# yinan-codes/Rossby-wave-ray-tracing

Measured on AMD Instinct MI355X. Metric: ray-steps/sec (whole node), 10^6 rays RKF45; max |Δpos| vs CPU ref, higher is better.
Workload: dtype f64

## Files before the change

include/rwrt.h:

```cpp
#ifndef RWRT_H
#define RWRT_H

#include <stdint.h>

#ifdef __cplusplus
extern "C" {
#endif

#define RWRT_ABI_VERSION 5
#define RWRT_NFIELD_REF 18
#define RWRT_NFIELD_PACK 12
#define RWRT_NVAR 5
#define RWRT_NMERC 12
#define RWRT_NOUT 8
#define RWRT_NSTATE 12

typedef enum {
  RWRT_OK = 0,
  RWRT_ERR_ARG = 1,
  RWRT_ERR_HIP = 2,
  RWRT_SOLVER_FAILED = 3
} rwrt_status;

typedef struct {
// ... 8 lines not shown
  double atol;
  double min_step;
  double cut_off;
  int32_t nt;
  int32_t reserved;
  double tstep;
} rwrt_params;

typedef struct {
  const void* d_levels;
  int32_t nlev;
  int32_t fp32;
  double t0;
  double dt;
} rwrt_background;
const char* rwrt_version(void);

typedef struct rwrt_ctx rwrt_ctx;
rwrt_status rwrt_ctx_create(int32_t device, rwrt_ctx** out);
rwrt_status rwrt_ctx_destroy(rwrt_ctx* ctx);
rwrt_status rwrt_ctx_set_latency_density(rwrt_ctx* ctx, int32_t rays_per_wave);
rwrt_status rwrt_ctx_set_tv_lanes(rwrt_ctx* ctx, int32_t lanes);
rwrt_status rwrt_ctx_set_handoff(rwrt_ctx* ctx, int32_t max_rays);
rwrt_status rwrt_ctx_set_trace(rwrt_ctx* ctx, int64_t* d_trace, int64_t capacity);
const char* rwrt_last_error(void);

rwrt_status rwrt_pack_fields(const rwrt_grid* g, const double* d_fields,
                             double* d_packed, void* stream);

rwrt_status rwrt_mercator_point(const rwrt_grid* g, const double* d_packed,
                                int64_t n, const double* d_lon,
                                const double* d_lat, double* d_out,
                                void* stream);

rwrt_status rwrt_rhs(const rwrt_grid* g, const double* d_packed, int64_t n,
                     const double* d_y, double* d_dydt, void* stream);

rwrt_status rwrt_dp54_attempt(const rwrt_grid* g, const double* d_packed,
                              int64_t n, const double* d_y, const double* d_f,
                              const double* d_h, double rtol, double atol,
                              double* d_K, double* d_ynew, double* d_err,
                              void* stream);

rwrt_status rwrt_ray_initial(const rwrt_grid* g, const double* d_packed,
                             int64_t nsource, const double* d_src_lon,
                             const double* d_src_lat, const double* d_src_cos,
// ... 246 lines not shown
```

rossby-wave-ray-tracing_amd/_hip.py:

```python
import ctypes
import os

import torch

_HERE = os.path.dirname(os.path.abspath(__file__))
LIB_PATH = os.environ.get("RWRT_LIB", os.path.join(_HERE, "librwrt.so"))

NFIELD_REF, NFIELD_PACK, NVAR, NMERC, NOUT, NSTATE = 18, 12, 5, 12, 8, 12
ABI_SYMBOLS = ("rwrt_version", "rwrt_last_error", "rwrt_ctx_create", "rwrt_ctx_destroy",
               "rwrt_ctx_set_latency_density", "rwrt_ctx_set_tv_lanes", "rwrt_ctx_set_handoff",
               "rwrt_ctx_set_trace",
               "rwrt_pack_fields",
               "rwrt_mercator_point", "rwrt_rhs", "rwrt_dp54_attempt",
               "rwrt_ray_initial", "rwrt_rk45_init", "rwrt_rk45_run", "rwrt_rk45_run_tails",
               "rwrt_expand_tails", "rwrt_row_slots", "rwrt_rk45_run_slots", "rwrt_expand_slots",
               "rwrt_launch_plan_bytes", "rwrt_launch_plan",
               "rwrt_rk4_run", "rwrt_ray_density", "rwrt_ray_summary", "rwrt_ray_arrival", "rwrt_ray_flux",
               "rwrt_ray_track", "rwrt_ray_cross",
               "rwrt_wn_map", "rwrt_wn_fill",
               "rwrt_sh_filter",
               "rwrt_bs_ready", "rwrt_bs_diag", "rwrt_rk45_init_tv", "rwrt_rk45_run_tv", "rwrt_rk45_run_tv_tails",
               "rwrt_rk45_run_tv_slots", "rwrt_rhs_tv",
               "rwrt_rk45_init_stack", "rwrt_rk45_run_stack",
               "rwrt_kat_rk45", "rwrt_selftest_math", "rwrt_host_fill_rows")

RWRT_OK, RWRT_ERR_ARG, RWRT_ERR_HIP, RWRT_SOLVER_FAILED = 0, 1, 2, 3
PLAN_SINCE, PLAN_TOTAL = 0, 1


class RwrtError(RuntimeError):
    pass


class SolverFailed(RwrtError):
# ... 129 lines not shown
        "rwrt_ray_track": [T, _I64, _I32, _I32, _P, _P, _P, _P, _P, _I64, _P, _P, _P, _P, _P, _P, _P],
        "rwrt_ray_cross": [X, _I64, _I32, _I32, _P, _P, _P, _P, _P, _I64, _P, _P, _P, _P, _P, _P, _P, _P, _P],
        "rwrt_ray_summary": [_I64, _I32, _I32, _P, _P, _P, _P, _P, _I64, R, _P, _P, _P],
        "rwrt_wn_map": [G, _P, _I32, _I64, _I32, _P, _P, _P, _I32, _P, _P, _P, _P, _P, _P, _P],
        "rwrt_wn_fill": [_I32, _I32, _I32, _I32, _P, _P, _P],
        "rwrt_sh_filter": [_I32, _I32, _I32, _I32, _P, _P, _P, _P, _P, _P, _P, _P],
        "rwrt_bs_ready": [_I32, _I32, _P, _P, _P, _D, _D, _P, _P, _I32, _P],
        "rwrt_bs_diag": [_I32, _I32, _I32, _P, _P, _P, _D, _D, ctypes.c_uint32, _P, _P, _I32, _P],
        "rwrt_rk45_init_tv": [G, B, _I64, _P, Pr, _P, _P, _P, _P, _P, _P],
        "rwrt_rk45_run_tv": [_P, G, B, _I64, Pr, _P, _I32, _I32, _P, _I64, _P, _P, _P, _P, _P, _P],
        "rwrt_rk45_run_tv_tails": [_P, G, B, _I64, Pr, _P, _I32, _I32, _P, _I64, _P, _P, _P, _P, _P, _P, _P,
                                   _P],
        "rwrt_rk45_run_tv_slots": [_P, G, B, _I64, Pr, _P, _I32, _I32, _P, _I64, _P, _P, _P, _P, _P, _P, _P,
                                   _P, _P],
        "rwrt_rk45_init_stack": [G, ctypes.POINTER(Stack), _I64, _P, Pr, _P, _P, _P, _P, _P, _P],
        "rwrt_rk45_run_stack": [_P, G, ctypes.POINTER(Stack), _I64, Pr, _P, _I32, _I32, _P, _P, _P, _P, _P, _P, _P,
                                _P, _P, _P],
        "rwrt_ctx_create": [_I32, ctypes.POINTER(_P)],
        "rwrt_ctx_destroy": [_P],
        "rwrt_ctx_set_latency_density": [_P, _I32],
        "rwrt_ctx_set_tv_lanes": [_P, _I32],
        "rwrt_ctx_set_handoff": [_P, _I32],
        "rwrt_ctx_set_trace": [_P, _P, _I64],
        "rwrt_rhs_tv": [G, B, _I64, _P, _P, _P, _P],
        "rwrt_kat_rk45": [_I32, _I64, _P, _I32, _P, _D, _D, _D, _P, _P],
        "rwrt_selftest_math": [_I32, _I64, _P, _P, _P, _P],
        "rwrt_host_fill_rows": [_P, _I64, _I64, _I64, _P, _P, _I64, _I64, _P],
    }
    for name, args in sig.items():
        fn = getattr(lib, name, None)
        if fn is None:
            continue
        fn.argtypes = args
        fn.restype = ctypes.c_int
    _lib = lib
    return lib


def version():
    return load().rwrt_version().decode()


def check(status):
    if status != RWRT_OK:
        msg = load().rwrt_last_error().decode()
        raise RwrtError(f"rwrt status {status}: {msg}")
# ... 29 lines not shown
        idx = self.device.index if self.device.index is not None else torch.cuda.current_device()
        h = _P()
        check(load().rwrt_ctx_create(int(idx), ctypes.byref(h)))
        self._h = h

    @property
    def handle(self):
        return self._h

    def set_latency_density(self, rays_per_wave):
        if getattr(self, "_qpw", 16) != int(rays_per_wave):
            check(load().rwrt_ctx_set_latency_density(self._h, int(rays_per_wave)))
            self._qpw = int(rays_per_wave)

    def set_tv_lanes(self, lanes):
        if getattr(self, "_tvl", 64) != int(lanes):
            check(load().rwrt_ctx_set_tv_lanes(self._h, int(lanes)))
            self._tvl = int(lanes)

    def set_handoff(self, max_rays):
        if getattr(self, "_hof", 16) != int(max_rays):
            check(load().rwrt_ctx_set_handoff(self._h, int(max_rays)))
            self._hof = int(max_rays)

    def set_trace(self, trace=None):
        if trace is None:
            check(load().rwrt_ctx_set_trace(self._h, None, 0))
        else:
            check(load().rwrt_ctx_set_trace(self._h, ctypes.c_void_p(trace.data_ptr()), int(trace.shape[0])))
        self._trace = trace

    _plan_scratch = None
    _plan_rays = 0

    def launch_plan(self, nray, total, state, count, prev_work, work, order, row_slot, nslot):
        lib = load()
        if self._plan_scratch is None or self._plan_rays < nray:
            need = _I64()
            check(lib.rwrt_launch_plan_bytes(int(nray), ctypes.byref(need)))
            self._plan_scratch = torch.empty(need.value, dtype=torch.uint8, device=self.device)
            self._plan_rays = int(nray)
        n_live = _I64()
        i64 = torch.int64
        check(lib.rwrt_launch_plan(int(nray), PLAN_TOTAL if total else PLAN_SINCE, dptr(state), dptr(count, i64),
                                   dptr(prev_work, i64), dptr(work, i64), dptr(order, i64),
                                   dptr(row_slot, torch.int32), dptr(nslot, i64), ctypes.byref(n_live),
# ... 14 lines not shown
```

rossby-wave-ray-tracing_amd/csrc/rwrt.hip:

```cpp

#include <hip/hip_runtime.h>

#include <cmath>
#include <cstdint>
#include <cstdlib>
#include <cstdio>
#include <cstring>
#include <mutex>
#include <string>
#include <type_traits>

#include "rwrt.h"
#include "nproots.h"

#ifdef RWRT_ANALYZE_HOT
__device__ __forceinline__ bool rwrt_rare_sink(bool c) {
  asm volatile("; rare %0" ::"s"(__builtin_amdgcn_ballot_w64(c)));
  return false;
}
#define RARE(c) rwrt_rare_sink(c)
#else
#define RARE(c) (c)
#endif
#ifdef RWRT_ANALYZE_MARK
#define MARK(name) do { __builtin_amdgcn_sched_barrier(0); asm volatile("; @MARK " name); __builtin_amdgcn_sched_barrier(0); } while (0)
#else
#define MARK(name)
#endif

#include "ray_point.h"
#include "stack_image.h"

namespace rwrt {

constexpr double kREarth = 6.3712e6;
constexpr double kOmega = 7.2921e-5;

__device__ __forceinline__ double div_rearth(double x) { return x / kREarth; }

#ifndef RWRT_ROW_NT
#define RWRT_ROW_NT 0
#endif
typedef double v2f64 __attribute__((ext_vector_type(2)));
template <bool NT>
__device__ __forceinline__ void store_row16(double2* o, double2 v) {
  if (NT) {
    v2f64 w;
    w.x = v.x;
    w.y = v.y;
    __builtin_nontemporal_store(w, reinterpret_cast<v2f64*>(o));
  } else {
    *o = v;
  }
// ... 2091 lines not shown
  int32_t handoff = 16;
};

template <class BG>
__device__ __forceinline__ double* row_block(const RunArgs<BG>& a, int64_t ray) {
  const int64_t slot = a.row_slot ? (int64_t)a.row_slot[ray] : ray;
  return slot < 0 ? nullptr : a.out + (size_t)slot * (size_t)(a.it_end - a.it_begin) * RWRT_NOUT;
}


__device__ __forceinline__ void store_tail(double* tail_row, int64_t ray, double2 r0, double2 r1, double2 r2,
                                           double2 r3) {
  double2* o = reinterpret_cast<double2*>(tail_row + (size_t)ray * RWRT_NOUT);
  o[0] = r0;
  o[1] = r1;
  o[2] = r2;
  o[3] = r3;
}

constexpr int kFlagHead = 256;
template <class BG>
__device__ __forceinline__ double* last_rows(const RunArgs<BG>& a) {
  return *reinterpret_cast<double* const*>(a.frozen - kFlagHead);
}

constexpr int kTraceWords = 10;
__device__ __forceinline__ void trace_start(int64_t* tr, int64_t w) {
  tr[w * kTraceWords + 3] = (int64_t)__builtin_amdgcn_s_memrealtime();
  tr[w * kTraceWords + 8] = (int64_t)__builtin_amdgcn_s_memtime();
}
__device__ __forceinline__ void trace_ray(int64_t* tr, int64_t w, int64_t ray, int64_t attempts, bool latency) {
  const unsigned hw = __builtin_amdgcn_s_getreg(4 | (31 << 11));
  const unsigned xcc = __builtin_amdgcn_s_getreg(20 | (15 << 11));
  int64_t* r = tr + w * kTraceWords;
  r[0] = ray;
  r[1] = hw;
  r[2] = xcc;
  r[4] = (int64_t)__builtin_amdgcn_s_memrealtime();
  r[5] = attempts;
  r[6] = latency ? 1 : 0;
  r[7] = blockIdx.x;
  r[9] = (int64_t)__builtin_amdgcn_s_memtime();
}

inline double haversine_cut(double cut_off) {
  if (!(cut_off > 0.0 && cut_off <= 3.0)) return -1.0;
// ... 397 lines not shown
  if (kTrace && w < a.trace_cap && R.role == 0) trace_start(a.trace, w);
  int32_t nanrow = a.nanrow[ray];
  int32_t it = a.it_begin;
  double prev_lon = y[0], prev_lat = y[1], cos_prev = k_cos(prev_lat);
  aux[2] = kNaN;
  bool in_step = false, rejected = false;
  quad_run<kTrace>(a, B, R, K, ray, rows, y, f, aux, t, habs, hs, nacc, nrej, att0, nanrow, it, prev_lon,
                   prev_lat, cos_prev, in_step, rejected, w);
}

using KStore = KShared<5>;
#ifndef RWRT_RUN_ALIGN
#define RWRT_RUN_ALIGN 256
#endif
template <class BG>
struct TvBlock {
  using type = void;
};
template <class T>
struct TvBlock<VaryingBG<T>> {
  using type = BlockVaryingBG<T>;
};

template <class BG, class LBG, bool kTrace, bool kReplica, bool kPair = false>
__device__ __forceinline__ void run_rays(const RunArgs<BG>& a, const LBG& lbg, char* smem, int64_t hw) {
  using RayProblem = RayProblemT<LBG>;
  const RayProblem P{lbg};
  const bool writer = kReplica ? (threadIdx.x & 63u) == 0 : kPair ? (threadIdx.x & 63u) < 32u : true;
  Lane<RayProblem, KStore> L;
  L.K.p = reinterpret_cast<double*>(smem) + threadIdx.x;
  L.K.stride = 256;
  int64_t ray = -1, nacc = 0, nrej = 0;
  double* rows = nullptr;
  int32_t it = 0, nanrow = 0, wpos = 0;
  double prev_lon = 0.0, prev_lat = 0.0, cos_prev = 0.0;
  constexpr bool kHandoff = std::is_base_of<CachedStaticBG, LBG>::value && !kReplica && !kPair && !kTrace;
  bool handoff = false;
  __builtin_amdgcn_s_setprio(1);
  for (;;) {
    if (ray < 0) {
      int64_t w;
      if (kReplica) {
        if (hw < 0) break;
        w = hw;
        hw = -1;
      } else if (kPair) {
        int64_t w0 = 0;
        if ((threadIdx.x & 63u) < 32u) w0 = a.n_heavy + atomicAdd(&a.queue[1], 1);
        w = __shfl(w0, (int)(threadIdx.x & 31u));
      } else {
        w = a.n_heavy + atomicAdd(&a.queue[1], 1);
      }
      if (w >= a.nray) break;
      ray = a.order ? a.order[w] : w;
      if (kTrace) {
        wpos = (int32_t)w;
        if (w < a.trace_cap) trace_start(a.trace, w);
      }
      if (a.frozen && a.frozen[ray]) {
        ray = -1;
        continue;
      }
      if constexpr (std::is_same<LBG, CachedStackBG>::value) P.B.pull(a.B, ray);
#pragma unroll
      for (int v = 0; v < 5; ++v) {
        L.y[v] = a.state[v * a.nray + ray];
        L.f[v] = a.state[(5 + v) * a.nray + ray];
      }
      L.t = a.state[10 * a.nray + ray];
      L.habs = a.state[11 * a.nray + ray];
      rows = row_block(a, ray);
      L.in_step = false;
      L.rejected = false;
      L.hs = 0.0;
      nacc = a.count[2 * ray];
      nrej = a.count[2 * ray + 1];
      nanrow = a.nanrow[ray];
      it = a.it_begin;
      prev_lon = L.y[0];
      prev_lat = L.y[1];
      cos_prev = k_cos(prev_lat);
      L.aux[2] = kNaN;
    }
    if constexpr (kHandoff) {
      if (RARE(__builtin_popcountll(__builtin_amdgcn_ballot_w64(true)) <= (unsigned)a.handoff)) {
        const int32_t q = __atomic_load_n(&a.queue[1], __ATOMIC_RELAXED);
        if (a.n_heavy + (int64_t)q >= a.nray) {
          handoff = true;
          break;
        }
      }
    }
    const double tb = a.tbound[it];
    const int st = L.iterate(P, tb, a.min_step, a.rtol, a.atol, nacc, nrej);
    if (st == Lane<RayProblem, KStore>::kStep) continue;
    MARK("x_row_end");

    double* y = L.y;
#ifndef RWRT_TV_REUSE_K6
#define RWRT_TV_REUSE_K6 1
#endif
    const bool have = (!BG::kTimeVarying || (RWRT_TV_REUSE_K6 && L.tk6 == tb)) && !isnan(L.aux[2]);
    double ug, vg, cos_c = kNaN;
    bool masked = fabs(y[1]) >= kHalfPi;
    if (!masked) {
      cos_c = L.aux[2];
      if (RARE(!have)) cos_c = cos_small(y[1]);
      masked = cal_dis_reaches(y[0], y[1], prev_lon, prev_lat, cos_c, cos_prev, a.cut_off, a.cut_a);
    }
    if (masked) {
// ... 124 lines not shown
      if (w >= a.n_heavy) return;
      using BBG = typename TvBlock<BG>::type;
      run_rays<BG, BBG, false, true>(a, BBG::make(a.B, smem + kKBytes), smem, w);
      return;
    }
  }
  if constexpr (std::is_same<BG, VaryingBG<double>>::value) {
#ifdef RWRT_ANALYZE_PAIR
    if (true) {
#else
    if (a.B.half) {
#endif
      run_rays<BG, PairVaryingBG64, false, false, true>(a, PairVaryingBG64::make(a.B, smem + kKBytes), smem, -1);
      return;
    }
  }
  if constexpr (kLean)
    run_rays<BG, LeanCachedStaticBG, kTrace, false>(a, LeanCachedStaticBG{LaneBG<BG>::make(a.B, smem + kKBytes)}, smem,
                                                    -1);
  else
    run_rays<BG, typename LaneBG<BG>::type, kTrace, false>(a, LaneBG<BG>::make(a.B, smem + kKBytes), smem, -1);
}

__global__ void frozen_flag_kernel(const double* __restrict__ state, int64_t nray,
                                   uint8_t* __restrict__ frozen, int32_t* __restrict__ tail_from = nullptr,
                                   int32_t it_begin = 0, int32_t it_end = 0, double* tail_row = nullptr) {
  if (blockIdx.x == 0 && threadIdx.x == 0) *reinterpret_cast<double**>(frozen - kFlagHead) = tail_row;
  for (int64_t i = blockIdx.x * (int64_t)blockDim.x + threadIdx.x; i < nray;
       i += (int64_t)gridDim.x * blockDim.x) {
    double sum = state[i];
#pragma unroll
    for (int v = 1; v < 5; ++v) sum = sum + state[v * nray + i];
    const bool frz = isnan(sum / 5.0);
    frozen[i] = frz ? 1 : 0;
    if (tail_from) tail_from[i] = frz ? it_begin : it_end;
  }
}

constexpr int kFillThreads = 64;
__device__ __forceinline__ void write_frozen_tile(double* out, int64_t base, int64_t nrows, bool mine,
                                                  double2 r0, double2 r1, double2 r2, double2 r3) {
  unsigned long long lanes = __ballot(mine);
  const int64_t nq = nrows * 4;
  const int qt = threadIdx.x & 3;
  while (lanes) {
    const int j = __builtin_ctzll(lanes);
    lanes &= lanes - 1;
    double2* o = reinterpret_cast<double2*>(out + (size_t)(base + j) * nrows * RWRT_NOUT);
    const double2 q0 = make_double2(__shfl(r0.x, j), __shfl(r0.y, j));
    const double2 q1 = make_double2(__shfl(r1.x, j), __shfl(r1.y, j));
// ... 443 lines not shown
  InitArgs<BG> a{B, nray, d_y0, p->rtol, p->atol, p->nt, d_state, d_count, d_nanrow, d_live, d_summary};
  hipLaunchKernelGGL(rk45_init_kernel<BG>, dim3(grid_for(nray, 256)), dim3(256), 0,
                     (hipStream_t)stream, a);
  return check_launch("rk45_init_kernel");
}

}

struct rwrt_ctx {
  int device = 0;
  int ncu = 256;
  int blocks_static = 0, blocks_f32 = 0, blocks_f64 = 0, blocks_a32 = 0;
  int blocks_stack = 0;
  uint8_t* flags = nullptr;
  size_t cap = 0;
  char* img = nullptr;
  size_t img_cap = 0;
  hipStream_t side = nullptr;
  hipEvent_t flagged = nullptr, filled = nullptr;
  hipEvent_t done = nullptr;
  int quad_per_wave = 16;
  int tv_lanes = 64;
  int handoff = 16;
  int64_t* trace = nullptr;
  int64_t trace_cap = 0;
  bool used = false;
  std::mutex mu;
};

namespace rwrt {

struct DeviceGuard {
  int prev = -1;
  bool ok = true;
  explicit DeviceGuard(int dev) {
    if (hipGetDevice(&prev) != hipSuccess) prev = -1;
    if (prev != dev) ok = hipSetDevice(dev) == hipSuccess;
  }
  ~DeviceGuard() {
    int cur = -1;
    if (prev >= 0 && hipGetDevice(&cur) == hipSuccess && cur != prev) (void)hipSetDevice(prev);
  }
};

rwrt_status ctx_flags(rwrt_ctx* c, int64_t nray) {
  if ((size_t)nray <= c->cap) return RWRT_OK;
// ... 107 lines not shown
                       int32_t* d_work, void* stream, const int32_t* d_row_slot = nullptr) {
  if (rwrt_status s = ctx_check(ctx)) return s;
  if (!p) return fail(RWRT_ERR_ARG, "params is NULL%s");
  if (nray < 0 || nray > 0x7fffffffLL) return fail(RWRT_ERR_ARG, "nray out of range%s");
  if (it_begin < 1 || it_end > p->nt || it_begin >= it_end)
    return fail(RWRT_ERR_ARG, "need 1 <= it_begin < it_end <= nt%s");
  if (!d_tbound || !d_work || (nray > 0 && (!d_state || !d_count || !d_nanrow || !d_out)))
    return fail(RWRT_ERR_ARG, "NULL buffer to rwrt_rk45_run%s");
  if (reinterpret_cast<uintptr_t>(d_out) % 16 != 0)
    return fail(RWRT_ERR_ARG, "output rows must be 16-byte aligned%s");
  if (!d_tail_from != !d_tail_row) return fail(RWRT_ERR_ARG, "tails need both d_tail_from and d_tail_row%s");
  if (reinterpret_cast<uintptr_t>(d_tail_row) % 16 != 0)
    return fail(RWRT_ERR_ARG, "tail rows must be 16-byte aligned%s");
  if (d_row_slot && !d_tail_from)
    return fail(RWRT_ERR_ARG, "row slots need tails (the rays without a slot keep theirs there)%s");
  if (nray == 0) return RWRT_OK;
  if (n_heavy < 0 || n_heavy > nray) return fail(RWRT_ERR_ARG, "n_heavy out of range%s");
  if (n_heavy > 0 && !d_order) return fail(RWRT_ERR_ARG, "n_heavy > 0 needs d_order%s");
  if (n_heavy > 0 && std::is_void<typename TvBlock<BG>::type>::value && !std::is_same<BG, StaticBG>::value)
    return fail(RWRT_ERR_ARG, "latency mode (n_heavy > 0) is not built for fp32-arithmetic levels%s");
  std::lock_guard<std::mutex> lock(ctx->mu);
  const int32_t quad_per_wave = ctx->quad_per_wave;
  const int32_t handoff = ctx->handoff;
  const int64_t per_block = BG::kTimeVarying ? 4 : 4 * (int64_t)quad_per_wave;
  const int64_t team_blocks = (n_heavy + per_block - 1) / per_block;
  if (team_blocks > ctx->ncu / 2)
    return fail(RWRT_ERR_ARG, "n_heavy exceeds the latency mode's capacity (per CU 4 x rays-per-wave, time-varying 4; half the CUs)%s");
  DeviceGuard dg(ctx->device);
  if (!dg.ok) return check_launch("hipSetDevice(context device)");
  hipStream_t st = (hipStream_t)stream;
  if (hipMemsetAsync(d_work, 0, 2 * sizeof(int32_t), st) != hipSuccess)
    return check_launch("hipMemsetAsync(queue)");
  int64_t blocks = ctx_persistent_blocks<BG>(ctx);
  if (team_blocks) blocks = std::max<int64_t>(1, blocks - team_blocks * (blocks / ctx->ncu));
  int64_t block_rays = 256;
  if constexpr (BG::kTimeVarying) block_rays = B.half ? 128 : 256;
  const int64_t need = (nray - n_heavy + block_rays - 1) / block_rays;
  if (blocks > need) blocks = need;
  RunArgs<BG> a{B, nray, p->rtol, p->atol, p->min_step, p->cut_off, p->nt, it_begin, it_end,
                d_tbound, d_order, d_state, d_count, d_nanrow, d_out, d_work,
                n_heavy, 0, haversine_cut(p->cut_off), nullptr};
  a.row_slot = d_row_slot;
  a.handoff = handoff;
  if (rwrt_status s = ctx_flags(ctx, nray)) return s;
  a.frozen = ctx->flags + kFlagHead;
  if (rwrt_status s = ctx_begin(ctx, st, [&] {
        hipLaunchKernelGGL(frozen_flag_kernel, dim3(grid_for(nray, 256)), dim3(256), 0, st, d_state, nray,
                           ctx->flags + kFlagHead, d_tail_from, it_begin, it_end, d_tail_row);
      }))
    return s;
  if constexpr (std::is_same<BG, StaticBG>::value) {
    if (rwrt_status s = ctx_image(ctx, B.F, st, &a.B.img, &a.B.range)) return s;
  }
  if constexpr (std::is_same<BG, StackBG>::value) {
    if (rwrt_status s = ctx_stack_images(ctx, B, st, &a.B.img)) return s;
  }
  a.heavy_blocks = (int32_t)team_blocks;
  a.quad_per_wave = quad_per_wave;
  if constexpr (std::is_same<BG, StaticBG>::value) {
    a.trace = ctx->trace;
    a.trace_cap = ctx->trace ? ctx->trace_cap : 0;
  }
  if (nray > n_heavy || team_blocks) {
    const int64_t grid = team_blocks + (nray > n_heavy ? blocks : 0);
    if (a.trace && std::is_same<BG, StaticBG>::value) {
      if constexpr (std::is_same<BG, StaticBG>::value) {
        hipLaunchKernelGGL((rk45_run_kernel<BG, true>), dim3((unsigned)grid), dim3(256), 0, st, a);
        hipLaunchKernelGGL((rk45_run_kernel<BG, true, true>), dim3((unsigned)grid), dim3(256), 0, st, a);
      }
    } else {
      hipLaunchKernelGGL(rk45_run_kernel<BG>, dim3((unsigned)grid), dim3(256), 0, st, a);
      if constexpr (std::is_same<BG, StaticBG>::value)
        hipLaunchKernelGGL((rk45_run_kernel<BG, false, true>), dim3((unsigned)grid), dim3(256), 0, st, a);
    }
    if (rwrt_status s = check_launch("rk45_run_kernel")) return s;
  }
  if (d_tail_from)
    hipLaunchKernelGGL(frozen_tail_kernel<BG>, dim3((unsigned)((nray + kFillThreads - 1) / kFillThreads)),
                       dim3(kFillThreads), 0, ctx->side, a, d_tail_row);
  else
    hipLaunchKernelGGL(frozen_fill_kernel<BG>, dim3((unsigned)((nray + kFillThreads - 1) / kFillThreads)),
                       dim3(kFillThreads), 0, ctx->side, a);
  if (rwrt_status s = check_launch(d_tail_from ? "frozen_tail_kernel" : "frozen_fill_kernel")) return s;
  return ctx_end(ctx, st);
}

template <class T>
rwrt_status make_varying(const rwrt_grid* g, const rwrt_background* b, VaryingBG<T>& B) {
  Field F;
  if (!b) return fail(RWRT_ERR_ARG, "background is NULL%s");
  if (rwrt_status s = make_field(g, reinterpret_cast<const double*>(b->d_levels), F)) return s;
  if (b->nlev < 1) return fail(RWRT_ERR_ARG, "background needs nlev >= 1%s");
  if (!(b->dt > 0.0)) return fail(RWRT_ERR_ARG, "background level spacing dt must be > 0%s");
  B.P = reinterpret_cast<const T*>(b->d_levels);
  B.W = F.W;
  B.H = F.H;
  B.nlev = b->nlev;
  B.lev_stride = (int64_t)F.W * F.H * kNF;
// ... 255 lines not shown
using namespace rwrt;

extern "C" {

const char* rwrt_version(void) { return "rwrt 0.5 (gfx950, abi 5)"; }

rwrt_status rwrt_ctx_create(int32_t device, rwrt_ctx** out) {
  if (!out) return fail(RWRT_ERR_ARG, "out is NULL%s");
  *out = nullptr;
  int ndev = 0;
  if (hipGetDeviceCount(&ndev) != hipSuccess || device < 0 || device >= ndev)
    return fail(RWRT_ERR_ARG, "no such HIP device%s");
  DeviceGuard dg(device);
  if (!dg.ok) return check_launch("hipSetDevice");
  rwrt_ctx* c = new (std::nothrow) rwrt_ctx;
  if (!c) return fail(RWRT_ERR_HIP, "out of host memory%s");
  c->device = device;
  int ncu = 0;
  if (hipDeviceGetAttribute(&ncu, hipDeviceAttributeMultiprocessorCount, device) == hipSuccess && ncu > 0)
    c->ncu = ncu;
  if (hipStreamCreateWithFlags(&c->side, hipStreamNonBlocking) != hipSuccess ||
      hipEventCreateWithFlags(&c->flagged, hipEventDisableTiming) != hipSuccess ||
      hipEventCreateWithFlags(&c->filled, hipEventDisableTiming) != hipSuccess ||
      hipEventCreateWithFlags(&c->done, hipEventDisableTiming) != hipSuccess) {
    rwrt_status s = check_launch("creating the context's stream and events");
    rwrt_ctx_destroy(c);
    return s ? s : fail(RWRT_ERR_HIP, "creating the context's stream and events failed%s");
  }
  *out = c;
  return RWRT_OK;
}

rwrt_status rwrt_ctx_set_latency_density(rwrt_ctx* c, int32_t rays_per_wave) {
  if (!c) return fail(RWRT_ERR_ARG, "rwrt_ctx is NULL%s");
  if (rays_per_wave < 1 || rays_per_wave > 16) return fail(RWRT_ERR_ARG, "rays_per_wave must be 1..16%s");
  std::lock_guard<std::mutex> lock(c->mu);
  c->quad_per_wave = rays_per_wave;
  return RWRT_OK;
}

rwrt_status rwrt_ctx_set_tv_lanes(rwrt_ctx* c, int32_t lanes) {
  if (!c) return fail(RWRT_ERR_ARG, "rwrt_ctx is NULL%s");
  if (lanes != 32 && lanes != 64) return fail(RWRT_ERR_ARG, "time-varying lanes per wave must be 32 or 64%s");
  std::lock_guard<std::mutex> lock(c->mu);
  c->tv_lanes = lanes;
  return RWRT_OK;
}

rwrt_status rwrt_ctx_set_handoff(rwrt_ctx* ctx, int32_t max_rays) {
  if (rwrt_status s = ctx_check(ctx)) return s;
  if (max_rays < 0 || max_rays > 16) return fail(RWRT_ERR_ARG, "hand-off threshold must be 0..16 rays%s");
  std::lock_guard<std::mutex> lock(ctx->mu);
  ctx->handoff = max_rays;
  return RWRT_OK;
}

rwrt_status rwrt_ctx_set_trace(rwrt_ctx* c, int64_t* d_trace, int64_t capacity) {
  if (!c) return fail(RWRT_ERR_ARG, "rwrt_ctx is NULL%s");
  if (capacity < 0 || (capacity > 0 && !d_trace) || capacity > 0x7fffffffLL)
    return fail(RWRT_ERR_ARG, "trace capacity out of range or NULL trace buffer%s");
  std::lock_guard<std::mutex> lock(c->mu);
  c->trace = capacity ? d_trace : nullptr;
  c->trace_cap = capacity;
  return RWRT_OK;
}

rwrt_status rwrt_ctx_destroy(rwrt_ctx* c) {
  if (!c) return RWRT_OK;
  rwrt_status s = RWRT_OK;
  {
    std::lock_guard<std::mutex> lock(c->mu);
    DeviceGuard dg(c->device);
    if (c->used && hipEventSynchronize(c->done) != hipSuccess) s = check_launch("rwrt_ctx_destroy");
    if (c->flags) (void)hipFree(c->flags);
    if (c->img) (void)hipFree(c->img);
    if (c->side) (void)hipStreamDestroy(c->side);
    if (c->flagged) (void)hipEventDestroy(c->flagged);
    if (c->filled) (void)hipEventDestroy(c->filled);
    if (c->done) (void)hipEventDestroy(c->done);
  }
  delete c;
  return s;
}

const char* rwrt_last_error(void) { return g_err.c_str(); }

rwrt_status rwrt_pack_fields(const rwrt_grid* g, const double* d_fields, double* d_packed,
                             void* stream) {
  if (!g || !d_fields || !d_packed) return fail(RWRT_ERR_ARG, "NULL argument to rwrt_pack_fields%s");
  const int64_t npts = (int64_t)g->ncol * g->nrow;
  hipLaunchKernelGGL(pack_fields_kernel, dim3(grid_for(npts, 256)), dim3(256), 0,
                     (hipStream_t)stream, d_fields, d_packed, npts);
  return check_launch("pack_fields_kernel");
}

rwrt_status rwrt_mercator_point(const rwrt_grid* g, const double* d_packed, int64_t n,
                                const double* d_lon, const double* d_lat, double* d_out,
                                void* stream) {
  Field F;
// ... 413 lines not shown
```

rossby-wave-ray-tracing_amd/engine.py:

```python
import os

import numpy as np
import torch

import _hip as H
from constants import rearth as R_EARTH
from launch_rows import deliver

F64 = torch.float64


def grid_of(lon, lat, ncol):
    lon = np.asarray(lon, np.float64)
    lat = np.asarray(lat, np.float64)
    return H.Grid(int(ncol), len(lat), float(lon[0]), float(lon[1] - lon[0]),
                  float(lat[0]), float(lat[1] - lat[0]))


def t_eval_of(nt, tstep, ttotal=None):
    t = np.arange(nt) * np.float64(tstep)
    if ttotal is not None and t[-1] > ttotal:
        t[-1] = ttotal
    return t

# ... 47 lines not shown
        return self

    def count(self):
        self.n = int(self.n_dev.item())
        return self.n

    def last_row(self, view, tails, i1):
        if LAST_ROWS:
            return tails.row
        blk = view[self.slot.clamp(min=0).to(torch.int64), -1] if view.shape[0] else tails.row
        return torch.where((tails.frm < i1)[:, None], tails.row, blk)

    def dense(self, view, tails, i0, i1, out=None):
        nray = self.slot.numel()
        if out is None or out.numel() < nray * (i1 - i0) * H.NOUT:
            out = torch.empty((nray, i1 - i0, H.NOUT), dtype=F64, device=self.slot.device)
        d = out.reshape(-1)[: nray * (i1 - i0) * H.NOUT].view(nray, i1 - i0, H.NOUT)
        H.check(H.load().rwrt_expand_slots(nray, int(i0), int(i1), H.dptr(self.slot, torch.int32),
                                           H.dptr(tails.frm, torch.int32), H.dptr(tails.row, F64),
                                           H.dptr(view, F64), H.dptr(d, F64), H.stream(self.slot.device)))
        return d


class RayEngine:

    use_tails = os.environ.get("RWRT_TAILS", "1") != "0"
    tv_lanes = int(os.environ.get("RWRT_TV_LANES", "32"))
    use_slots = os.environ.get("RWRT_SLOTS", "1") != "0"
    handoff = int(os.environ.get("RWRT_HANDOFF", "16"))
    use_plan = os.environ.get("RWRT_PLAN", "1") != "0"

    def __init__(self, fields, lon, lat, device=None):
        H.require_gpu()
        H.load()
        self.device = torch.device(device or "cuda")
        f = torch.as_tensor(np.ascontiguousarray(fields, dtype=np.float64)) \
            if not torch.is_tensor(fields) else fields.to(F64)
        if f.ndim != 3 or f.shape[-1] != H.NFIELD_REF:
            raise ValueError(f"fields must be [ncol, nrow, {H.NFIELD_REF}], got {tuple(f.shape)}")
        f = f.to(self.device).contiguous()
        self.grid = grid_of(lon, lat, f.shape[0])
        self.lon, self.lat = np.array(lon, np.float64), np.array(lat, np.float64)
        self.packed = torch.empty((f.shape[0], f.shape[1], H.NFIELD_PACK), dtype=F64,
                                  device=self.device)
        H.check(H.load().rwrt_pack_fields(self.grid, H.dptr(f), H.dptr(self.packed), self._stream()))
        self.work = torch.zeros(4, dtype=torch.int32, device=self.device)

    bg = None
    nmember = 0
    split_rho = None
    launch_log = ()
    rows_bytes = 0
    launch_handoffs = ()
# ... 324 lines not shown
        return n_best, q_best

    def team_fixed(self, team, n_live):
        if self.bg is not None and self.bg.fp32 == 2:
            return 0, 16
        ncu = torch.cuda.get_device_properties(self.device).multi_processor_count
        n, q = (int(team[0]), int(team[1])) if isinstance(team, (tuple, list)) else (int(team), 16)
        return min(n, (ncu // 2) * 4 * (1 if self.bg is not None else q), n_live), q

    def plan_buffers(self, nray):
        return {"work": torch.empty(nray, dtype=torch.int64, device=self.device),
                "order": torch.empty(nray, dtype=torch.int64, device=self.device),
                "slots": Slots(nray, self.device)}

    def run(self, st, p, tbound, it_begin, it_end, out, order=None, n_heavy=0, rays_per_wave=16, tails=None,
            slots=None):
        lib = H.load()
        ctx = self.ctx
        if self.bg is not None:
            ctx.set_tv_lanes(self.tv_lanes)
        if n_heavy:
            ctx.set_latency_density(rays_per_wave)
        ctx.set_handoff(self.handoff)
        if slots is not None and tails is None:
            raise ValueError("row slots need tails")
        if self.nmember:
            if n_heavy:
                raise ValueError("member stacks have no latency mode (n_heavy must be 0)")
            stack = self.stack_of(st)
            H.check(lib.rwrt_rk45_run_stack(
                ctx.handle, self.grid, ctypes_ref(stack), st["nray"], ctypes_ref(p), H.dptr(tbound, F64),
                int(it_begin), int(it_end), H.dptr(order, torch.int64), H.dptr(st["state"]), H.dptr(st["count"]),
                H.dptr(st["nanrow"]), H.dptr(out, F64), None if slots is None else H.dptr(slots.slot, torch.int32),
                None if tails is None else H.dptr(tails.frm, torch.int32),
                None if tails is None else H.dptr(tails.row, F64), H.dptr(self.work), self._stream()))
            return
        if self.bg is None:
            fn, bg = (lib.rwrt_rk45_run if tails is None else lib.rwrt_rk45_run_tails if slots is None
                      else lib.rwrt_rk45_run_slots), H.dptr(self.packed)
        else:
            fn, bg = (lib.rwrt_rk45_run_tv if tails is None else lib.rwrt_rk45_run_tv_tails if slots is None
                      else lib.rwrt_rk45_run_tv_slots), ctypes_ref(self.bg)
        args = [ctx.handle, self.grid, bg, st["nray"], ctypes_ref(p), H.dptr(tbound, F64),
                int(it_begin), int(it_end), H.dptr(order, torch.int64), int(n_heavy),
                H.dptr(st["state"]), H.dptr(st["count"]), H.dptr(st["nanrow"]), H.dptr(out, F64)]
        if slots is not None:
# ... 373 lines not shown
```

Before: 4.224 billion.

## Add two-ended claim queue and optional concurrent lean kernel on a side stream

Ray claiming for the static background becomes wave-aggregated: one lane does a single 64-bit atomic on a packed head/tail counter and hands indices to the other lanes. This replaces the per-lane atomicAdd on the old queue. It also adds an optional lean-kernel path, off by default. That path computes the live queue end, then launches low-priority kernels on a separate stream that claim rays from the back of the queue while the main kernel takes them from the front, so the two overlap. The change adds new context state, a stage buffer, events, and a CAS loop for back claims.

```diff
diff --git a/include/rwrt.h b/include/rwrt.h
--- a/include/rwrt.h
+++ b/include/rwrt.h
@@ -54,6 +54,9 @@
 rwrt_status rwrt_ctx_set_latency_density(rwrt_ctx* ctx, int32_t rays_per_wave);
 rwrt_status rwrt_ctx_set_tv_lanes(rwrt_ctx* ctx, int32_t lanes);
 rwrt_status rwrt_ctx_set_handoff(rwrt_ctx* ctx, int32_t max_rays);
+rwrt_status rwrt_ctx_set_lean(rwrt_ctx* ctx, double share, int32_t min_rows);
+rwrt_status rwrt_ctx_set_lean_only(rwrt_ctx* ctx);
+rwrt_status rwrt_ctx_queue_ends(rwrt_ctx* ctx, int64_t* h_ends);
 rwrt_status rwrt_ctx_set_trace(rwrt_ctx* ctx, int64_t* d_trace, int64_t capacity);
 const char* rwrt_last_error(void);
 
diff --git a/rossby-wave-ray-tracing_amd/_hip.py b/rossby-wave-ray-tracing_amd/_hip.py
--- a/rossby-wave-ray-tracing_amd/_hip.py
+++ b/rossby-wave-ray-tracing_amd/_hip.py
@@ -9,7 +9,7 @@
 NFIELD_REF, NFIELD_PACK, NVAR, NMERC, NOUT, NSTATE = 18, 12, 5, 12, 8, 12
 ABI_SYMBOLS = ("rwrt_version", "rwrt_last_error", "rwrt_ctx_create", "rwrt_ctx_destroy",
                "rwrt_ctx_set_latency_density", "rwrt_ctx_set_tv_lanes", "rwrt_ctx_set_handoff",
-               "rwrt_ctx_set_trace",
+               "rwrt_ctx_set_trace", "rwrt_ctx_set_lean", "rwrt_ctx_set_lean_only", "rwrt_ctx_queue_ends",
                "rwrt_pack_fields",
                "rwrt_mercator_point", "rwrt_rhs", "rwrt_dp54_attempt",
                "rwrt_ray_initial", "rwrt_rk45_init", "rwrt_rk45_run", "rwrt_rk45_run_tails",
@@ -185,6 +185,9 @@
         "rwrt_ctx_set_tv_lanes": [_P, _I32],
         "rwrt_ctx_set_handoff": [_P, _I32],
         "rwrt_ctx_set_trace": [_P, _P, _I64],
+        "rwrt_ctx_set_lean": [_P, _D, _I32],
+        "rwrt_ctx_set_lean_only": [_P],
+        "rwrt_ctx_queue_ends": [_P, _P],
         "rwrt_rhs_tv": [G, B, _I64, _P, _P, _P, _P],
         "rwrt_kat_rk45": [_I32, _I64, _P, _I32, _P, _D, _D, _D, _P, _P],
         "rwrt_selftest_math": [_I32, _I64, _P, _P, _P, _P],
@@ -260,6 +263,20 @@
         if getattr(self, "_hof", 16) != int(max_rays):
             check(load().rwrt_ctx_set_handoff(self._h, int(max_rays)))
             self._hof = int(max_rays)
+
+    def set_lean(self, share, min_rows=0):
+        key = (share, int(min_rows))
+        if getattr(self, "_lean", (0.0, 0)) != key:
+            if share == "only":
+                check(load().rwrt_ctx_set_lean_only(self._h))
+            else:
+                check(load().rwrt_ctx_set_lean(self._h, float(share), int(min_rows)))
+            self._lean = key
+
+    def queue_ends(self):
+        ends = (_I64 * 3)()
+        check(load().rwrt_ctx_queue_ends(self._h, ends))
+        return int(ends[0]), int(ends[1]), int(ends[2])
 
     def set_trace(self, trace=None):
         if trace is None:
diff --git a/rossby-wave-ray-tracing_amd/csrc/claim_queue.h b/rossby-wave-ray-tracing_amd/csrc/claim_queue.h
--- /dev/null
+++ b/rossby-wave-ray-tracing_amd/csrc/claim_queue.h
@@ -0,0 +1,34 @@
+#ifndef RWRT_CLAIM_QUEUE_H
+#define RWRT_CLAIM_QUEUE_H
+#include <cstdint>
+
+#if defined(__HIPCC__) || defined(__CUDACC__)
+#define RWRT_CQ_FN __host__ __device__ inline
+#else
+#define RWRT_CQ_FN inline
+#endif
+
+namespace rwrt {
+namespace claimq {
+
+constexpr uint64_t kFront = 1ull;
+constexpr uint64_t kBack = 1ull << 32;
+
+RWRT_CQ_FN uint32_t head(uint64_t v) { return (uint32_t)v; }
+RWRT_CQ_FN uint32_t tail(uint64_t v) { return (uint32_t)(v >> 32); }
+RWRT_CQ_FN int64_t taken(uint64_t v) { return (int64_t)head(v) + (int64_t)tail(v); }
+
+RWRT_CQ_FN int64_t front_position(uint64_t old, int64_t n) {
+  return taken(old) < n ? (int64_t)head(old) : -1;
+}
+
+RWRT_CQ_FN int64_t back_room(uint64_t cur, int64_t n, int64_t stop) {
+  const int64_t room = (n < stop ? n : stop) - taken(cur);
+  return room > 0 ? room : 0;
+}
+RWRT_CQ_FN bool back_open(uint64_t cur, int64_t n, int64_t stop) { return back_room(cur, n, stop) > 0; }
+RWRT_CQ_FN int64_t back_position(uint64_t cur, int64_t n) { return n - 1 - (int64_t)tail(cur); }
+
+}
+}
+#endif
diff --git a/rossby-wave-ray-tracing_amd/csrc/rwrt.hip b/rossby-wave-ray-tracing_amd/csrc/rwrt.hip
--- a/rossby-wave-ray-tracing_amd/csrc/rwrt.hip
+++ b/rossby-wave-ray-tracing_amd/csrc/rwrt.hip
@@ -29,6 +29,7 @@
 #endif
 
 #include "ray_point.h"
+#include "claim_queue.h"
 #include "stack_image.h"
 
 namespace rwrt {
@@ -2166,6 +2167,63 @@
 template <class BG>
 __device__ __forceinline__ double* last_rows(const RunArgs<BG>& a) {
   return *reinterpret_cast<double* const*>(a.frozen - kFlagHead);
+}
+constexpr int kHeadQueueLen = 1, kHeadLeanShare = 2, kHeadClaims = 16;
+static_assert((kHeadClaims + 1) * 8 <= kFlagHead, "the header holds the claim counter");
+template <class BG>
+__device__ __forceinline__ int64_t queue_len(const RunArgs<BG>& a) {
+  return reinterpret_cast<const int64_t*>(a.frozen - kFlagHead)[kHeadQueueLen];
+}
+template <class BG>
+__device__ __forceinline__ unsigned long long* queue_claims(const RunArgs<BG>& a) {
+  return reinterpret_cast<unsigned long long*>(const_cast<uint8_t*>(a.frozen) - kFlagHead) + kHeadClaims;
+}
+struct ClaimLanes {
+  uint64_t lanes;
+  unsigned rank;
+  __device__ __forceinline__ ClaimLanes() {
+    lanes = __builtin_amdgcn_ballot_w64(true);
+    rank = __builtin_amdgcn_mbcnt_hi((uint32_t)(lanes >> 32), __builtin_amdgcn_mbcnt_lo((uint32_t)lanes, 0u));
+  }
+  __device__ __forceinline__ unsigned count() const { return (unsigned)__builtin_popcountll(lanes); }
+  __device__ __forceinline__ uint64_t first(uint64_t v) const {
+    const uint32_t lo = __builtin_amdgcn_readfirstlane((uint32_t)v);
+    const uint32_t hi = __builtin_amdgcn_readfirstlane((uint32_t)(v >> 32));
+    return ((uint64_t)hi << 32) | lo;
+  }
+};
+template <class BG>
+__device__ __forceinline__ int64_t claim_front(const RunArgs<BG>& a) {
+  const ClaimLanes L;
+  uint64_t old = 0;
+  if (L.rank == 0) old = atomicAdd(queue_claims(a), (unsigned long long)(L.count() * claimq::kFront));
+  old = L.first(old) + L.rank * claimq::kFront;
+  const int64_t q = claimq::front_position(old, queue_len(a));
+  return q < 0 ? -1 : a.n_heavy + q;
+}
+template <class BG>
+__device__ __forceinline__ int64_t claim_back(const RunArgs<BG>& a, int64_t stop) {
+  const ClaimLanes L;
+  const int64_t n = queue_len(a);
+  uint64_t cur = 0, got = 0;
+  if (L.rank == 0) {
+    unsigned long long* const c = queue_claims(a);
+    cur = __atomic_load_n(c, __ATOMIC_RELAXED);
+    for (;;) {
+      const int64_t room = claimq::back_room(cur, n, stop);
+      if (room <= 0) break;
+      const uint64_t k = room < (int64_t)L.count() ? (uint64_t)room : (uint64_t)L.count();
+      const uint64_t seen = atomicCAS(c, (unsigned long long)cur, (unsigned long long)(cur + k * claimq::kBack));
+      if (seen == cur) {
+        got = k;
+        break;
+      }
+      cur = seen;
+    }
+  }
+  cur = L.first(cur);
+  got = L.first(got);
+  return L.rank < got ? a.n_heavy + claimq::back_position(cur, n) - (int64_t)L.rank : -1;
 }
 
 constexpr int kTraceWords = 10;
@@ -2609,8 +2667,9 @@
   using type = BlockVaryingBG<T>;
 };
 
-template <class BG, class LBG, bool kTrace, bool kReplica, bool kPair = false>
-__device__ __forceinline__ void run_rays(const RunArgs<BG>& a, const LBG& lbg, char* smem, int64_t hw) {
+template <class BG, class LBG, bool kTrace, bool kReplica, bool kPair = false, bool kBack = false>
+__device__ __forceinline__ void run_rays(const RunArgs<BG>& a, const LBG& lbg, char* smem, int64_t hw,
+                                         int64_t lean_stop = 0) {
   using RayProblem = RayProblemT<LBG>;
   const RayProblem P{lbg};
   const bool writer = kReplica ? (threadIdx.x & 63u) == 0 : kPair ? (threadIdx.x & 63u) < 32u : true;
@@ -2623,7 +2682,7 @@
   double prev_lon = 0.0, prev_lat = 0.0, cos_prev = 0.0;
   constexpr bool kHandoff = std::is_base_of<CachedStaticBG, LBG>::value && !kReplica && !kPair && !kTrace;
   bool handoff = false;
-  __builtin_amdgcn_s_setprio(1);
+  if constexpr (!kBack) __builtin_amdgcn_s_setprio(1);
   for (;;) {
     if (ray < 0) {
       int64_t w;
@@ -2635,6 +2694,12 @@
         int64_t w0 = 0;
         if ((threadIdx.x & 63u) < 32u) w0 = a.n_heavy + atomicAdd(&a.queue[1], 1);
         w = __shfl(w0, (int)(threadIdx.x & 31u));
+      } else if constexpr (kBack) {
+        w = claim_back(a, lean_stop);
+        if (w < 0) break;
+      } else if constexpr (std::is_same<BG, StaticBG>::value) {
+        w = claim_front(a);
+        if (w < 0) break;
       } else {
         w = a.n_heavy + atomicAdd(&a.queue[1], 1);
       }
@@ -2671,8 +2736,8 @@
     }
     if constexpr (kHandoff) {
       if (RARE(__builtin_popcountll(__builtin_amdgcn_ballot_w64(true)) <= (unsigned)a.handoff)) {
-        const int32_t q = __atomic_load_n(&a.queue[1], __ATOMIC_RELAXED);
-        if (a.n_heavy + (int64_t)q >= a.nray) {
+        const uint64_t q = __atomic_load_n(queue_claims(a), __ATOMIC_RELAXED);
+        if (claimq::taken(q) >= queue_len(a)) {
           handoff = true;
           break;
         }
@@ -2843,10 +2908,47 @@
     run_rays<BG, typename LaneBG<BG>::type, kTrace, false>(a, LaneBG<BG>::make(a.B, smem + kKBytes), smem, -1);
 }
 
+constexpr int kLeanStageDoubles = 5 * 5 * 256;
+template <bool kLean>
+__global__ void __launch_bounds__(256) __attribute__((amdgpu_waves_per_eu(4, 4)))
+rk45_lean_kernel(RunArgs<StaticBG> a, double* __restrict__ stages) {
+#ifndef RWRT_ANALYZE_HOT
+  if (bg_lean(a.B.range, a.B.F) != kLean) return;
+#endif
+  nm_stage<NM_ALL>();
+  const double share = reinterpret_cast<const double*>(a.frozen - kFlagHead)[kHeadLeanShare];
+  const int64_t stop = (int64_t)(share * (double)queue_len(a));
+  char* const slice = reinterpret_cast<char*>(stages + (size_t)blockIdx.x * kLeanStageDoubles);
+  using LBG = typename std::conditional<kLean, LeanStaticBG, StaticBG>::type;
+  run_rays<StaticBG, LBG, false, false, false, true>(a, LBG{a.B}, slice, -1, stop);
+}
+
+__global__ void queue_end_kernel(const int64_t* __restrict__ order, const uint8_t* __restrict__ frozen,
+                                 int64_t nray, int64_t n_heavy) {
+  int64_t end = 0;
+  for (int64_t w = n_heavy + blockIdx.x * (int64_t)blockDim.x + threadIdx.x; w < nray;
+       w += (int64_t)gridDim.x * blockDim.x)
+    if (!frozen[order ? order[w] : w]) end = w + 1 - n_heavy;
+#pragma unroll
+  for (int d = 32; d > 0; d >>= 1) {
+    const int64_t o = (int64_t)__shfl_xor((long long)end, d);
+    end = o > end ? o : end;
+  }
+  if ((threadIdx.x & 63u) == 0 && end > 0)
+    atomicMax(reinterpret_cast<long long*>(const_cast<uint8_t*>(frozen) - kFlagHead) + kHeadQueueLen, (long long)end);
+}
+
 __global__ void frozen_flag_kernel(const double* __restrict__ state, int64_t nray,
                                    uint8_t* __restrict__ frozen, int32_t* __restrict__ tail_from = nullptr,
-                                   int32_t it_begin = 0, int32_t it_end = 0, double* tail_row = nullptr) {
-  if (blockIdx.x == 0 && threadIdx.x == 0) *reinterpret_cast<double**>(frozen - kFlagHead) = tail_row;
+                                   int32_t it_begin = 0, int32_t it_end = 0, double* tail_row = nullptr,
+                                   int64_t queue_len = 0, double lean_share = 0.0) {
+  if (blockIdx.x == 0 && threadIdx.x == 0) {
+    *reinterpret_cast<double**>(frozen - kFlagHead) = tail_row;
+    int64_t* const h = reinterpret_cast<int64_t*>(frozen - kFlagHead);
+    h[kHeadQueueLen] = queue_len;
+    h[kHeadClaims] = 0;
+    reinterpret_cast<double*>(h)[kHeadLeanShare] = lean_share;
+  }
   for (int64_t i = blockIdx.x * (int64_t)blockDim.x + threadIdx.x; i < nray;
        i += (int64_t)gridDim.x * blockDim.x) {
     double sum = state[i];
@@ -3336,6 +3438,13 @@
   int quad_per_wave = 16;
   int tv_lanes = 64;
   int handoff = 16;
+  hipStream_t lean = nullptr;
+  hipEvent_t imaged = nullptr, leaned = nullptr;
+  double* lean_stages = nullptr;
+  int lean_blocks = 0;
+  double lean_share = 0.0;
+  int lean_min_rows = 0;
+  bool lean_only = false;
   int64_t* trace = nullptr;
   int64_t trace_cap = 0;
   bool used = false;
@@ -3489,6 +3598,10 @@
   std::lock_guard<std::mutex> lock(ctx->mu);
   const int32_t quad_per_wave = ctx->quad_per_wave;
   const int32_t handoff = ctx->handoff;
+  const bool lean = std::is_same<BG, StaticBG>::value && ctx->lean_share > 0.0 &&
+                    it_end - it_begin >= ctx->lean_min_rows && nray > n_heavy && !ctx->trace;
+  const bool lean_only = lean && ctx->lean_only;
+  const double lean_share = lean ? ctx->lean_share : 0.0;
   const int64_t per_block = BG::kTimeVarying ? 4 : 4 * (int64_t)quad_per_wave;
   const int64_t team_blocks = (n_heavy + per_block - 1) / per_block;
   if (team_blocks > ctx->ncu / 2)
@@ -3513,11 +3626,30 @@
   a.frozen = ctx->flags + kFlagHead;
   if (rwrt_status s = ctx_begin(ctx, st, [&] {
         hipLaunchKernelGGL(frozen_flag_kernel, dim3(grid_for(nray, 256)), dim3(256), 0, st, d_state, nray,
-                           ctx->flags + kFlagHead, d_tail_from, it_begin, it_end, d_tail_row);
+                           ctx->flags + kFlagHead, d_tail_from, it_begin, it_end, d_tail_row,
+                           lean ? (int64_t)0 : nray - n_heavy, lean_share);
       }))
     return s;
   if constexpr (std::is_same<BG, StaticBG>::value) {
     if (rwrt_status s = ctx_image(ctx, B.F, st, &a.B.img, &a.B.range)) return s;
+    if (lean) {
+      if (!ctx->lean_stages || ctx->lean_blocks < blocks) {
+        if (ctx->lean_stages &&
+            ((ctx->used && hipEventSynchronize(ctx->done) != hipSuccess) || hipFree(ctx->lean_stages) != hipSuccess))
+          return check_launch("releasing the context's lean stage buffer");
+        ctx->lean_stages = nullptr;
+        ctx->lean_blocks = 0;
+        if (hipMalloc(reinterpret_cast<void**>(&ctx->lean_stages),
+                      (size_t)blocks * kLeanStageDoubles * sizeof(double)) != hipSuccess)
+          return fail(RWRT_ERR_HIP, "lean stage buffer allocation failed%s");
+        ctx->lean_blocks = (int)blocks;
+      }
+      hipLaunchKernelGGL(queue_end_kernel, dim3(grid_for(nray - n_heavy, 256)), dim3(256), 0, st, d_order,
+                         ctx->flags + kFlagHead, nray, n_heavy);
+      if (rwrt_status s = check_launch("queue_end_kernel")) return s;
+      if (hipEventRecord(ctx->imaged, st) != hipSuccess || hipStreamWaitEvent(ctx->lean, ctx->imaged, 0) != hipSuccess)
+        return check_launch("hipEventRecord(lean pair)");
+    }
   }
   if constexpr (std::is_same<BG, StackBG>::value) {
     if (rwrt_status s = ctx_stack_images(ctx, B, st, &a.B.img)) return s;
@@ -3528,8 +3660,8 @@
     a.trace = ctx->trace;
     a.trace_cap = ctx->trace ? ctx->trace_cap : 0;
   }
-  if (nray > n_heavy || team_blocks) {
-    const int64_t grid = team_blocks + (nray > n_heavy ? blocks : 0);
+  if ((nray > n_heavy && !lean_only) || team_blocks) {
+    const int64_t grid = team_blocks + (nray > n_heavy && !lean_only ? blocks : 0);
     if (a.trace && std::is_same<BG, StaticBG>::value) {
       if constexpr (std::is_same<BG, StaticBG>::value) {
         hipLaunchKernelGGL((rk45_run_kernel<BG, true>), dim3((unsigned)grid), dim3(256), 0, st, a);
@@ -3541,6 +3673,15 @@
         hipLaunchKernelGGL((rk45_run_kernel<BG, false, true>), dim3((unsigned)grid), dim3(256), 0, st, a);
     }
     if (rwrt_status s = check_launch("rk45_run_kernel")) return s;
+  }
+  if constexpr (std::is_same<BG, StaticBG>::value) {
+    if (lean) {
+      hipLaunchKernelGGL(rk45_lean_kernel<false>, dim3((unsigned)blocks), dim3(256), 0, ctx->lean, a, ctx->lean_stages);
+      hipLaunchKernelGGL(rk45_lean_kernel<true>, dim3((unsigned)blocks), dim3(256), 0, ctx->lean, a, ctx->lean_stages);
+      if (rwrt_status s = check_launch("rk45_lean_kernel")) return s;
+      if (hipEventRecord(ctx->leaned, ctx->lean) != hipSuccess || hipStreamWaitEvent(st, ctx->leaned, 0) != hipSuccess)
+        return check_launch("hipEventRecord(lean pair's end)");
+    }
   }
   if (d_tail_from)
     hipLaunchKernelGGL(frozen_tail_kernel<BG>, dim3((unsigned)((nray + kFillThreads - 1) / kFillThreads)),
@@ -3842,7 +3983,10 @@
   if (hipStreamCreateWithFlags(&c->side, hipStreamNonBlocking) != hipSuccess ||
       hipEventCreateWithFlags(&c->flagged, hipEventDisableTiming) != hipSuccess ||
       hipEventCreateWithFlags(&c->filled, hipEventDisableTiming) != hipSuccess ||
-      hipEventCreateWithFlags(&c->done, hipEventDisableTiming) != hipSuccess) {
+      hipEventCreateWithFlags(&c->done, hipEventDisableTiming) != hipSuccess ||
+      hipStreamCreateWithFlags(&c->lean, hipStreamNonBlocking) != hipSuccess ||
+      hipEventCreateWithFlags(&c->imaged, hipEventDisableTiming) != hipSuccess ||
+      hipEventCreateWithFlags(&c->leaned, hipEventDisableTiming) != hipSuccess) {
     rwrt_status s = check_launch("creating the context's stream and events");
     rwrt_ctx_destroy(c);
     return s ? s : fail(RWRT_ERR_HIP, "creating the context's stream and events failed%s");
@@ -3872,6 +4016,45 @@
   if (max_rays < 0 || max_rays > 16) return fail(RWRT_ERR_ARG, "hand-off threshold must be 0..16 rays%s");
   std::lock_guard<std::mutex> lock(ctx->mu);
   ctx->handoff = max_rays;
+  return RWRT_OK;
+}
+
+rwrt_status rwrt_ctx_set_lean(rwrt_ctx* ctx, double share, int32_t min_rows) {
+  if (rwrt_status s = ctx_check(ctx)) return s;
+  if (!(share >= 0.0 && share <= 1.0) || min_rows < 0)
+    return fail(RWRT_ERR_ARG, "lean share must be 0..1 and min_rows >= 0%s");
+  std::lock_guard<std::mutex> lock(ctx->mu);
+  ctx->lean_share = share;
+  ctx->lean_min_rows = min_rows;
+  ctx->lean_only = false;
+  return RWRT_OK;
+}
+
+rwrt_status rwrt_ctx_set_lean_only(rwrt_ctx* ctx) {
+  if (rwrt_status s = ctx_check(ctx)) return s;
+  std::lock_guard<std::mutex> lock(ctx->mu);
+  ctx->lean_share = 1.0;
+  ctx->lean_min_rows = 0;
+  ctx->lean_only = true;
+  return RWRT_OK;
+}
+
+rwrt_status rwrt_ctx_queue_ends(rwrt_ctx* ctx, int64_t* h_ends) {
+  if (rwrt_status s = ctx_check(ctx)) return s;
+  if (!h_ends) return fail(RWRT_ERR_ARG, "h_ends is NULL%s");
+  std::lock_guard<std::mutex> lock(ctx->mu);
+  h_ends[0] = h_ends[1] = h_ends[2] = 0;
+  if (!ctx->used || !ctx->flags) return RWRT_OK;
+  DeviceGuard dg(ctx->device);
+  if (!dg.ok) return check_launch("hipSetDevice(context device)");
+  int64_t h[kHeadClaims + 1];
+  if (hipEventSynchronize(ctx->done) != hipSuccess ||
+      hipMemcpy(h, ctx->flags, sizeof(h), hipMemcpyDeviceToHost) != hipSuccess)
+    return check_launch("reading the context's queue");
+  const uint64_t c = (uint64_t)h[kHeadClaims];
+  h_ends[2] = h[kHeadQueueLen];
+  h_ends[1] = (int64_t)claimq::tail(c);
+  h_ends[0] = h_ends[2] - h_ends[1];
   return RWRT_OK;
 }
 
@@ -3894,7 +4077,11 @@
     if (c->used && hipEventSynchronize(c->done) != hipSuccess) s = check_launch("rwrt_ctx_destroy");
     if (c->flags) (void)hipFree(c->flags);
     if (c->img) (void)hipFree(c->img);
+    if (c->lean_stages) (void)hipFree(c->lean_stages);
     if (c->side) (void)hipStreamDestroy(c->side);
+    if (c->lean) (void)hipStreamDestroy(c->lean);
+    if (c->imaged) (void)hipEventDestroy(c->imaged);
+    if (c->leaned) (void)hipEventDestroy(c->leaned);
     if (c->flagged) (void)hipEventDestroy(c->flagged);
     if (c->filled) (void)hipEventDestroy(c->filled);
     if (c->done) (void)hipEventDestroy(c->done);
diff --git a/rossby-wave-ray-tracing_amd/engine.py b/rossby-wave-ray-tracing_amd/engine.py
--- a/rossby-wave-ray-tracing_amd/engine.py
+++ b/rossby-wave-ray-tracing_amd/engine.py
@@ -93,6 +93,20 @@
         return d
 
 
+LEAN_DEFAULT = "0"
+
+
+def parse_lean(text):
+    text = str(text).strip()
+    if text == "only":
+        return ("only", 0)
+    share, _, rows = text.partition(":")
+    share, rows = float(share), int(rows or 0)
+    if not 0.0 <= share <= 1.0 or rows < 0:
+        raise ValueError(f"RWRT_LEAN: 0, only, share or share:min_rows with 0 <= share <= 1, not {text!r}")
+    return (share, rows)
+
+
 class RayEngine:
 
     use_tails = os.environ.get("RWRT_TAILS", "1") != "0"
@@ -100,6 +114,7 @@
     use_slots = os.environ.get("RWRT_SLOTS", "1") != "0"
     handoff = int(os.environ.get("RWRT_HANDOFF", "16"))
     use_plan = os.environ.get("RWRT_PLAN", "1") != "0"
+    lean = parse_lean(os.environ.get("RWRT_LEAN", LEAN_DEFAULT))
 
     def __init__(self, fields, lon, lat, device=None):
         H.require_gpu()
@@ -470,6 +485,7 @@
         if n_heavy:
             ctx.set_latency_density(rays_per_wave)
         ctx.set_handoff(self.handoff)
+        ctx.set_lean(*self.lean)
         if slots is not None and tails is None:
             raise ValueError("row slots need tails")
         if self.nmember:
```

Result: no change. 4.236 billion (median of 6 runs) (+0.3%).
